# roclark/torchsr

Measured on AMD Instinct MI355X. Metric: 96x96 HR crops/sec (SRGAN GAN train step), higher is better.
Workload: dtype f32; 1 GPU; SRGAN full GAN step (Generator + Discriminator + VGG19 perceptual loss), 96x96 HR crops, batch 16 per GPU, fp32; per_gpu_batch=16, global_batch=16, crop=96, parallelism=dp1, hip_graph=True, vgg19_weights=seeded-random, plan_cus=256

## Files before the change

### torchsr_amd/csrc/convpack.hip

```cpp
#include "conv_host.h"

namespace {

__global__ void pack_fwd_kernel(const float* __restrict__ w, float* __restrict__ p, int Cout, int Cin, int KH, int KW,
                                int Ck, int K, int Kp, int Cnp, int shuffle_cps) {
  const int64_t idx = (int64_t)blockIdx.x * blockDim.x + threadIdx.x;
  if (idx >= (int64_t)Cnp * Kp) return;
  const int np = (int)(idx / Kp), k = (int)(idx - (int64_t)np * Kp);
  float v = 0.f;
  if (np < Cout && k < K) {
    const int tap = k / Ck, ci = k - tap * Ck;
    if (ci < Cin) {
      int co = np;
      if (shuffle_cps) { const int ij = np / shuffle_cps, cc = np - ij * shuffle_cps; co = cc * 4 + ij; }
      const int kh = tap / KW, kw = tap - kh * KW;
      v = w[(((size_t)co * Cin + ci) * KH + kh) * KW + kw];
    }
  }
  p[idx] = v;
}

__global__ void pack_bwd_kernel(const float* __restrict__ w, float* __restrict__ p, int Cout, int Cin, int KH, int KW,
                                int stride, int pad, int ph, int pw, int dminh, int dminw, int ntw, int Ck, int K,
                                int Kp, int Cnp, int shuffle_cps) {
  const int64_t idx = (int64_t)blockIdx.x * blockDim.x + threadIdx.x;
  if (idx >= (int64_t)Cnp * Kp) return;
  const int ci = (int)(idx / Kp), k = (int)(idx - (int64_t)ci * Kp);
  float v = 0.f;
  if (ci < Cin && k < K) {
    const int tap = k / Ck, c = k - tap * Ck;
    if (c < Cout) {
      const int th = tap / ntw, tw = tap - th * ntw;
      const int kh = ph + pad - stride * (dminh + th), kw = pw + pad - stride * (dminw + tw);
      int co = c;
      if (shuffle_cps) { const int ij = c / shuffle_cps, cc = c - ij * shuffle_cps; co = cc * 4 + ij; }
      v = w[(((size_t)co * Cin + ci) * KH + kh) * KW + kw];
    }
  }
  p[idx] = v;
}

struct PackSeg { float* dst; int rows, K, Kp, Ck, bwd, ph, pw, dminh, dminw, ntw; };
struct PackArgs {
  const float* w;
  int Cout, Cin, KH, KW, stride, pad, cps, nseg;
  PackSeg seg[17];
};
__global__ void pack_all_kernel(const PackArgs a) {
  const PackSeg sg = a.seg[blockIdx.y];
  const int64_t idx = (int64_t)blockIdx.x * blockDim.x + threadIdx.x;
  if (idx >= (int64_t)sg.rows * sg.Kp) return;
  const int row = (int)(idx / sg.Kp), k = (int)(idx - (int64_t)row * sg.Kp);
  float v = 0.f;
  if (k < sg.K) {
    const int tap = k / sg.Ck, c = k - tap * sg.Ck;
    if (!sg.bwd) {
      if (row < a.Cout && c < a.Cin) {
        int co = row;
        if (a.cps) { const int ij = row / a.cps, cc = row - ij * a.cps; co = cc * 4 + ij; }
        const int kh = tap / a.KW, kw = tap - kh * a.KW;
        v = a.w[(((size_t)co * a.Cin + c) * a.KH + kh) * a.KW + kw];
      }
    } else {
      if (row < a.Cin && c < a.Cout) {
        const int th = tap / sg.ntw, tw = tap - th * sg.ntw;
        const int kh = sg.ph + a.pad - a.stride * (sg.dminh + th), kw = sg.pw + a.pad - a.stride * (sg.dminw + tw);
        int co = c;
        if (a.cps) { const int ij = c / a.cps, cc = c - ij * a.cps; co = cc * 4 + ij; }
        v = a.w[(((size_t)co * a.Cin + row) * a.KH + kh) * a.KW + kw];
      }
    }
  }
  sg.dst[idx] = v;
}

}

extern "C" int srx_conv2d_pack(const srx_conv2d_t* d, const float* w, float* wpk_fwd, float* wpk_bwd, void* stream) {
  if (int rc = check_desc(d)) return rc;
  SRX_REQUIRE(w && wpk_fwd, "conv2d_pack: null pointer");
  hipStream_t st = srx_stream(stream);
  const Geo g = fwd_geo(d);
  PackArgs pa{};
  pa.w = w; pa.Cout = d->Cout; pa.Cin = d->Cin; pa.KH = d->KH; pa.KW = d->KW; pa.stride = d->stride; pa.pad = d->pad;
  pa.cps = g.cps;
  int64_t maxn = 0;
  if (srx_thin_fwd_applicable(d)) {
    if (int rc = srx_thin_pack(d, w, wpk_fwd, 0, st)) return rc;
  } else {
    PackSeg& sg = pa.seg[pa.nseg++];
    sg = PackSeg{wpk_fwd, g.Cnp, g.K, g.Kp, g.Ck, 0, 0, 0, 0, 0, 1};
    maxn = (int64_t)g.Cnp * g.Kp;
  }
  if (wpk_bwd && srx_thin_dgrad_applicable(d)) {
    if (int rc = srx_thin_pack(d, w, wpk_bwd, 1, st)) return rc;
  } else if (wpk_bwd) {
    SRX_REQUIRE(d->stride <= 4, "conv2d_pack: stride > 4 unsupported for the data gradient");
    BwdClass cls[16];
    size_t total;
    const int nc = bwd_classes(d, cls, total);
    const int Ck = bwd_ck(d);
    const int Cnp = pad_rows(d->Cin);
    for (int i = 0; i < nc; ++i) {
      const BwdClass& c = cls[i];
      PackSeg& sg = pa.seg[pa.nseg++];
      sg = PackSeg{wpk_bwd + c.woff, Cnp, c.K, c.Kp, Ck, 1, c.ph, c.pw, c.dminh, c.dminw, c.ntw > 0 ? c.ntw : 1};
      if ((int64_t)Cnp * c.Kp > maxn) maxn = (int64_t)Cnp * c.Kp;
    }
  }
  if (pa.nseg > 0) {
    hipLaunchKernelGGL(pack_all_kernel, dim3((unsigned)srx_cdiv(maxn, 256), pa.nseg), dim3(256), 0, st, pa);
    SRX_CHECK_LAUNCH("pack_all_kernel");
  }
  return SRX_OK;
}

struct PackRec {
  float* dst; const float* w;
  long long n_elems;
  int kind;
  int rows, K, Kp, Ck, ph, pw, dminh, dminw, ntw;
  int Cout, Cin, KH, KW, stride, pad, cps, pad_;
};

__global__ void pack_table_kernel(const PackRec* __restrict__ table) {
  const PackRec r = table[blockIdx.y];
  const int64_t idx = (int64_t)blockIdx.x * blockDim.x + threadIdx.x;
  if (idx >= r.n_elems) return;
  float v = 0.f;
  if (r.kind >= 4) {
    srx_wino_pack_one(r.w, r.dst, r.Cout, r.Cin, r.kind == 5 ? 1 : (r.kind == 6 ? 2 : 0), idx);
    return;
  }
  if (r.kind >= 2) {
    const int taps = r.KH * r.KW;
    const int ch = (int)(idx & 63), tap = (int)((idx >> 6) % taps), c = (int)(idx / (64 * taps));
    const int Cthin = r.kind == 2 ? r.Cout : r.Cin;
    if (c < Cthin) {
      const int kh = tap / r.KW, kw = tap - kh * r.KW;
      v = r.kind == 2 ? r.w[(((size_t)c * 64 + ch) * r.KH + kh) * r.KW + kw]
                      : r.w[(((size_t)ch * Cthin + c) * r.KH + (r.KH - 1 - kh)) * r.KW + (r.KW - 1 - kw)];
    }
    r.dst[idx] = v;
    return;
  }
  const int taps = r.K / r.Ck;
  const int64_t nmain = (int64_t)r.rows * r.Ck;
  if (idx >= nmain) {
    const int padk = r.Kp - r.K;
    const int64_t j = idx - nmain;
    if (padk > 0 && j < (int64_t)r.rows * padk) {
      const int row = (int)(j / padk);
      r.dst[(size_t)row * r.Kp + r.K + (int)(j - (int64_t)row * padk)] = 0.f;
    }
    return;
  }
  const int row = (int)(idx / r.Ck), c = (int)(idx - (int64_t)row * r.Ck);
  float* d = r.dst + (size_t)row * r.Kp + c;
  const bool live = r.kind == 0 ? (row < r.Cout && c < r.Cin) : (row < r.Cin && c < r.Cout);
  int co = r.kind == 0 ? row : c;
  if (r.cps) { const int ij = co / r.cps, cc = co - ij * r.cps; co = cc * 4 + ij; }
  const float* src = r.w + ((size_t)co * r.Cin + (r.kind == 0 ? c : row)) * (r.KH * r.KW);
  for (int t0 = 0; t0 < taps; t0 += 9) {
    float v[9];
#pragma unroll
    for (int u = 0; u < 9; ++u) {
      const int tap = min(t0 + u, taps - 1);
      int off = tap;
      if (r.kind == 1) {
        const int th = tap / r.ntw, tw = tap - th * r.ntw;
        off = (r.ph + r.pad - r.stride * (r.dminh + th)) * r.KW + (r.pw + r.pad - r.stride * (r.dminw + tw));
      }
      v[u] = live ? src[off] : 0.f;
    }
#pragma unroll
    for (int u = 0; u < 9; ++u)
      if (t0 + u < taps) d[(size_t)(t0 + u) * r.Ck] = v[u];
  }
}

extern "C" size_t srx_pack_table_bytes(int n_layers) { return (size_t)n_layers * 17 * sizeof(PackRec); }

extern "C" int srx_pack_table_build(const srx_conv2d_t* descs, int n, const float* const* w, float* const* wpk_fwd,
                                    float* const* wpk_bwd, void* host_table, int* nrec_out, long long* max_elems_out) {
  SRX_REQUIRE(descs && w && wpk_fwd && wpk_bwd && host_table && nrec_out && max_elems_out && n > 0,
              "pack_table_build: bad argument");
  PackRec* out = static_cast<PackRec*>(host_table);
  int nrec = 0;
  long long maxn = 0;
  for (int i = 0; i < n; ++i) {
    const srx_conv2d_t* d = descs + i;
    if (int rc = check_desc(d)) return rc;
    SRX_REQUIRE(w[i] && wpk_fwd[i], "pack_table_build: null pointer in layer %d", i);
    const Geo g = fwd_geo(d);
    PackRec base{};
    base.w = w[i];
    base.Cout = d->Cout; base.Cin = d->Cin; base.KH = d->KH; base.KW = d->KW; base.stride = d->stride; base.pad = d->pad;
    base.cps = g.cps;
    auto emit = [&](PackRec r) {
      if (r.n_elems > maxn) maxn = r.n_elems;
      out[nrec++] = r;
    };
    if (srx_thin_fwd_applicable(d)) {
      PackRec r = base; r.kind = 2; r.dst = wpk_fwd[i]; r.n_elems = 4LL * d->KH * d->KW * 64; emit(r);
    } else {
      PackRec r = base; r.kind = 0; r.dst = wpk_fwd[i]; r.rows = g.Cnp; r.K = g.K; r.Kp = g.Kp; r.Ck = g.Ck; r.ntw = 1;
      r.n_elems = (long long)g.Cnp * (g.Ck + g.Kp - g.K); emit(r);
    }
    if (!wpk_bwd[i]) continue;
    if (srx_thin_dgrad_applicable(d)) {
      PackRec r = base; r.kind = 3; r.dst = wpk_bwd[i]; r.n_elems = 4LL * d->KH * d->KW * 64; emit(r);
      continue;
    }
    SRX_REQUIRE(d->stride <= 4, "pack_table_build: stride > 4 unsupported for the data gradient");
    BwdClass cls[16];
    size_t total;
    const int nc = bwd_classes(d, cls, total);
    const int Cnp = pad_rows(d->Cin);
    for (int c = 0; c < nc; ++c) {
      PackRec r = base; r.kind = 1; r.dst = wpk_bwd[i] + cls[c].woff;
      r.rows = Cnp; r.K = cls[c].K; r.Kp = cls[c].Kp; r.Ck = bwd_ck(d);
      r.ph = cls[c].ph; r.pw = cls[c].pw; r.dminh = cls[c].dminh; r.dminw = cls[c].dminw;
      r.ntw = cls[c].ntw > 0 ? cls[c].ntw : 1;
      r.n_elems = (long long)Cnp * (r.Ck + cls[c].Kp - cls[c].K);
      emit(r);
    }
  }
  *nrec_out = nrec;
  *max_elems_out = maxn;
  return SRX_OK;
}

extern "C" int srx_pack_table_add_wino(void* host_table, int* nrec, long long* max_elems, const srx_conv2d_t* d, const float* w,
                                       float* upk, int transpose) {
  SRX_REQUIRE(host_table && nrec && max_elems && d && w && upk && *nrec >= 0, "pack_table_add_wino: bad argument");
  SRX_REQUIRE(srx_wino_applicable(d) || srx_wino_packed_floats(d) > 0, "pack_table_add_wino: not a Winograd layer");
  PackRec r{};
  SRX_REQUIRE(!(transpose && d->shuffle), "pack_table_add_wino: a PixelShuffle layer has no Winograd data gradient");
  r.dst = upk; r.w = w; r.kind = transpose ? 5 : (d->shuffle ? 6 : 4);
  r.Cout = d->Cout; r.Cin = d->Cin; r.KH = 3; r.KW = 3; r.stride = 1; r.pad = 1;
  r.n_elems = (long long)d->Cout * d->Cin;
  static_cast<PackRec*>(host_table)[(*nrec)++] = r;
  if (r.n_elems > *max_elems) *max_elems = r.n_elems;
  return SRX_OK;
}

extern "C" int srx_pack_table_run(const void* dev_table, int nrec, long long max_elems, void* stream) {
  SRX_REQUIRE(dev_table && nrec > 0 && nrec <= 65535 && max_elems > 0, "pack_table_run: bad argument");
  hipLaunchKernelGGL(pack_table_kernel, dim3((unsigned)srx_cdiv(max_elems, 256), (unsigned)nrec), dim3(256), 0,
                     srx_stream(stream), static_cast<const PackRec*>(dev_table));
  SRX_CHECK_LAUNCH("pack_table_kernel");
  return SRX_OK;
}
```

Measured before the change: 2428 crops/s.

## Rework weight pack table kernel into LDS-tiled persistent grid with compact block schedule

Replaces the rectangular (max_elems x nrec) grid, in which most blocks exited idle, with a persistent 1D grid capped at 1024 blocks. Each block binary-searches a prefix-sum block table so the grid covers only real work. Dense forward and backward packs now stage contiguous weight runs through LDS and write 64-wide coalesced rows. Winograd packs now transform a 32x32 channel tile per block from LDS and use vector stores, instead of running one element per thread. This targets the strided, uncoalesced gather of the per-step weight repack, at the cost of more code complexity and LDS pressure.

Result: no change. 2427 crops/s (-0.1%).

```diff
diff --git a/torchsr_amd/csrc/convpack.hip b/torchsr_amd/csrc/convpack.hip
--- a/torchsr_amd/csrc/convpack.hip
+++ b/torchsr_amd/csrc/convpack.hip
@@ -120,18 +120,17 @@
   long long n_elems;
   int kind;
   int rows, K, Kp, Ck, ph, pw, dminh, dminw, ntw;
-  int Cout, Cin, KH, KW, stride, pad, cps, pad_;
+  int Cout, Cin, KH, KW, stride, pad, cps;
+  int blk0, nblk, rt;
 };
 
-__global__ void pack_table_kernel(const PackRec* __restrict__ table) {
-  const PackRec r = table[blockIdx.y];
-  const int64_t idx = (int64_t)blockIdx.x * blockDim.x + threadIdx.x;
+constexpr int PT_WPITCH = 32 * 9 + 1;
+constexpr int PT_LDS = 32 * PT_WPITCH;
+constexpr int PT_TAPS_MAX = (PT_LDS / 64 - 1);
+
+__device__ void pack_table_item(const PackRec& r, int64_t idx) {
   if (idx >= r.n_elems) return;
   float v = 0.f;
-  if (r.kind >= 4) {
-    srx_wino_pack_one(r.w, r.dst, r.Cout, r.Cin, r.kind == 5 ? 1 : (r.kind == 6 ? 2 : 0), idx);
-    return;
-  }
   if (r.kind >= 2) {
     const int taps = r.KH * r.KW;
     const int ch = (int)(idx & 63), tap = (int)((idx >> 6) % taps), c = (int)(idx / (64 * taps));
@@ -177,6 +176,149 @@
     for (int u = 0; u < 9; ++u)
       if (t0 + u < taps) d[(size_t)(t0 + u) * r.Ck] = v[u];
   }
+}
+
+__device__ __forceinline__ int pack_shuffled(int co, int cps) {
+  if (cps) { const int ij = co / cps, cc = co - ij * cps; co = cc * 4 + ij; }
+  return co;
+}
+
+template <class Src>
+__device__ __forceinline__ void pack_stage_runs(float* lds, int n, int len, int pitch, Src src) {
+  const int total = n * len;
+  for (int e0 = threadIdx.x; e0 < total; e0 += 18 * 256) {
+    float v[18];
+    int at[18];
+#pragma unroll
+    for (int u = 0; u < 18; ++u) {
+      const int e = min(e0 + u * 256, total - 1);
+      const int q = e / len, i = e - q * len;
+      at[u] = q * pitch + i;
+      v[u] = src(q)[i];
+    }
+#pragma unroll
+    for (int u = 0; u < 18; ++u)
+      if (e0 + u * 256 < total) lds[at[u]] = v[u];
+  }
+}
+
+__device__ void pack_table_tile(const PackRec& r, int lb, float* lds) {
+  const int T = r.KH * r.KW, taps = r.K / r.Ck;
+  const int nct = (r.Ck + 63) >> 6;
+  const int rtile = lb / nct, ct = lb - rtile * nct;
+  const int r0 = rtile * r.rt, c0 = ct * 64;
+  const int nr = min(r.rt, r.rows - r0), nc = min(64, r.Ck - c0);
+  const bool fwd = r.kind == 0;
+  const int lr = max(0, min(nr, (fwd ? r.Cout : r.Cin) - r0)), lc = max(0, min(nc, (fwd ? r.Cin : r.Cout) - c0));
+  const int pitch = fwd ? 64 * T : ((r.rt * T) | 1);
+  if (lr > 0 && lc > 0 && taps > 0) {
+    if (fwd) pack_stage_runs(lds, lr, lc * T, pitch, [&](int q) { return r.w + ((size_t)pack_shuffled(r0 + q, r.cps) * r.Cin + c0) * T; });
+    else     pack_stage_runs(lds, lc, lr * T, pitch, [&](int q) { return r.w + ((size_t)pack_shuffled(c0 + q, r.cps) * r.Cin + r0) * T; });
+  }
+  __syncthreads();
+  const int cc = threadIdx.x & 63;
+  if (cc < nc) {
+    for (int p = threadIdx.x >> 6; p < nr * taps; p += 4) {
+      const int rr = p / taps, tap = p - rr * taps;
+      int off = tap;
+      if (!fwd) {
+        const int th = tap / r.ntw, tw = tap - th * r.ntw;
+        off = (r.ph + r.pad - r.stride * (r.dminh + th)) * r.KW + (r.pw + r.pad - r.stride * (r.dminw + tw));
+      }
+      float v = 0.f;
+      if (rr < lr && cc < lc) v = fwd ? lds[rr * pitch + cc * T + off] : lds[cc * pitch + rr * T + off];
+      r.dst[(size_t)(r0 + rr) * r.Kp + (size_t)tap * r.Ck + c0 + cc] = v;
+    }
+  }
+  if (ct == 0) {
+    const int padk = r.Kp - r.K;
+    for (int j = threadIdx.x; j < nr * padk; j += 256) {
+      const int rr = j / padk;
+      r.dst[(size_t)(r0 + rr) * r.Kp + r.K + (j - rr * padk)] = 0.f;
+    }
+  }
+  __syncthreads();
+}
+
+__device__ void pack_table_wino_tile(const PackRec& r, int lb, float* lds) {
+  const bool tr = r.kind == 5;
+  const int R = tr ? r.Cin : r.Cout, K = tr ? r.Cout : r.Cin;
+  const int nch = K / 32, rt = R / 32;
+  const int jg = lb / nch, kc = lb - jg * nch;
+  const int q4 = r.Cout / 4;
+  if (tr) pack_stage_runs(lds, 32, 288, PT_WPITCH, [&](int q) { return r.w + ((size_t)(kc * 32 + q) * r.Cin + jg * 32) * 9; });
+  else    pack_stage_runs(lds, 32, 288, PT_WPITCH, [&](int q) {
+            const int row = jg * 32 + q;
+            return r.w + ((size_t)(r.kind == 6 ? (row % q4) * 4 + row / q4 : row) * r.Cin + kc * 32) * 9; });
+  __syncthreads();
+  const int s = threadIdx.x >> 6, hh = (threadIdx.x >> 5) & 1, mrow = threadIdx.x & 31;
+  float o[16][4];
+#pragma unroll
+  for (int e = 0; e < 4; ++e) {
+    const int kk = s * 8 + hh * 4 + e;
+    float g[3][3];
+#pragma unroll
+    for (int i = 0; i < 3; ++i)
+#pragma unroll
+      for (int j = 0; j < 3; ++j)
+        g[i][j] = tr ? lds[kk * PT_WPITCH + mrow * 9 + (2 - i) * 3 + (2 - j)] : lds[mrow * PT_WPITCH + kk * 9 + i * 3 + j];
+    float t[4][3];
+#pragma unroll
+    for (int j = 0; j < 3; ++j) {
+      t[0][j] = g[0][j];
+      t[1][j] = 0.5f * (g[0][j] + g[1][j] + g[2][j]);
+      t[2][j] = 0.5f * (g[0][j] - g[1][j] + g[2][j]);
+      t[3][j] = g[2][j];
+    }
+#pragma unroll
+    for (int i = 0; i < 4; ++i) {
+      const float u[4] = {t[i][0], 0.5f * (t[i][0] + t[i][1] + t[i][2]), 0.5f * (t[i][0] - t[i][1] + t[i][2]), t[i][2]};
+#pragma unroll
+      for (int j = 0; j < 4; ++j) o[4 * i + j][e] = u[j];
+    }
+  }
+  const bool whole = ((uintptr_t)r.dst & 15) == 0;
+#pragma unroll
+  for (int xi = 0; xi < 16; ++xi) {
+    float* d = r.dst + (((((size_t)xi * rt + jg) * nch + kc) * 4 + s) * 64 + hh * 32 + mrow) * 4;
+    if (whole) {
+      *reinterpret_cast<f32x4*>(d) = f32x4{o[xi][0], o[xi][1], o[xi][2], o[xi][3]};
+    } else {
+#pragma unroll
+      for (int e = 0; e < 4; ++e) d[e] = o[xi][e];
+    }
+  }
+  __syncthreads();
+}
+
+__global__ __launch_bounds__(256, 4) void pack_table_kernel(const PackRec* __restrict__ table, int nrec) {
+  __shared__ float lds[PT_LDS];
+  const int total = table[nrec - 1].blk0 + table[nrec - 1].nblk;
+  for (int vb = blockIdx.x; vb < total; vb += gridDim.x) {
+    int lo = 0, hi = nrec - 1;
+    while (lo < hi) {
+      const int mid = (lo + hi + 1) >> 1;
+      if (table[mid].blk0 <= vb) lo = mid; else hi = mid - 1;
+    }
+    const PackRec r = table[lo];
+    const int lb = vb - r.blk0;
+    if (r.kind >= 4) pack_table_wino_tile(r, lb, lds);
+    else if (r.kind < 2 && r.rt > 0) pack_table_tile(r, lb, lds);
+    else pack_table_item(r, (int64_t)lb * 256 + threadIdx.x);
+  }
+}
+
+static void pack_rec_place(PackRec& r, const PackRec* prev) {
+  r.rt = 0;
+  if (r.kind >= 4) {
+    r.nblk = (r.Cout / 32) * (r.Cin / 32);
+  } else if (r.kind < 2 && r.KH * r.KW <= PT_TAPS_MAX) {
+    r.rt = std::min(8, PT_TAPS_MAX / (r.KH * r.KW));
+    r.nblk = (int)(srx_cdiv(r.rows, r.rt) * srx_cdiv(r.Ck, 64));
+  } else {
+    r.nblk = (int)srx_cdiv(r.n_elems, 256);
+  }
+  r.blk0 = prev ? prev->blk0 + prev->nblk : 0;
 }
 
 extern "C" size_t srx_pack_table_bytes(int n_layers) { return (size_t)n_layers * 17 * sizeof(PackRec); }
@@ -199,6 +341,7 @@
     base.cps = g.cps;
     auto emit = [&](PackRec r) {
       if (r.n_elems > maxn) maxn = r.n_elems;
+      pack_rec_place(r, nrec ? out + nrec - 1 : nullptr);
       out[nrec++] = r;
     };
     if (srx_thin_fwd_applicable(d)) {
@@ -240,15 +383,18 @@
   r.dst = upk; r.w = w; r.kind = transpose ? 5 : (d->shuffle ? 6 : 4);
   r.Cout = d->Cout; r.Cin = d->Cin; r.KH = 3; r.KW = 3; r.stride = 1; r.pad = 1;
   r.n_elems = (long long)d->Cout * d->Cin;
-  static_cast<PackRec*>(host_table)[(*nrec)++] = r;
+  PackRec* tab = static_cast<PackRec*>(host_table);
+  pack_rec_place(r, *nrec ? tab + *nrec - 1 : nullptr);
+  tab[(*nrec)++] = r;
   if (r.n_elems > *max_elems) *max_elems = r.n_elems;
   return SRX_OK;
 }
 
 extern "C" int srx_pack_table_run(const void* dev_table, int nrec, long long max_elems, void* stream) {
   SRX_REQUIRE(dev_table && nrec > 0 && nrec <= 65535 && max_elems > 0, "pack_table_run: bad argument");
-  hipLaunchKernelGGL(pack_table_kernel, dim3((unsigned)srx_cdiv(max_elems, 256), (unsigned)nrec), dim3(256), 0,
-                     srx_stream(stream), static_cast<const PackRec*>(dev_table));
+  const int64_t blocks = std::min<int64_t>((int64_t)nrec * 4 * srx_cdiv(max_elems, 256), 1024);
+  hipLaunchKernelGGL(pack_table_kernel, dim3((unsigned)blocks), dim3(256), 0, srx_stream(stream),
+                     static_cast<const PackRec*>(dev_table), nrec);
   SRX_CHECK_LAUNCH("pack_table_kernel");
   return SRX_OK;
 }
```
